# ShiqiYu/libfacedetection.train

Hardware: AMD Instinct MI355X
Metric: training images/sec, YuNet_n 320x320 bs=256/GPU (higher is better)
Workload: dtype f32; 1 GPU; YuNet_n 320x320 bs=256/GPU full training step, fp32 (64->64 backward GEMMs: two-way bf16 split -- measured against the exact-fp32 instruction: every output within 9e-6 of its tensor maximum, 50 SGD iterations end as far from the exact path as a last-bit perturbation of it does, tests/test_precision_gpu.py + profiles/r05_precision.json; the strictly-fp32 variant is timed in exact_fp32_bwd with --fu; parallelism=dp1, global_batch=256

## Files before the change

### libfacedetection.train_amd/csrc/common.h

```cpp
#pragma once
#include <hip/hip_runtime.h>
#include <stdint.h>
#include <stdlib.h>

#include "../../include/yunet_hip.h"

#define CONV_BLOCKS 1024

typedef float f32x4 __attribute__((ext_vector_type(4)));
typedef unsigned int u32x4 __attribute__((ext_vector_type(4)));
typedef unsigned int u32x2 __attribute__((ext_vector_type(2)));

#ifdef YUNET_ACT_BF16
typedef unsigned short act_t;
typedef u32x2 act_raw4;
#define ACT_SUFFIX(name) name##_bf16
#define YUNET_ACT_DTYPE YUNET_BF16
#else
typedef float act_t;
typedef u32x4 act_raw4;
#define ACT_SUFFIX(name) name
#define YUNET_ACT_DTYPE YUNET_F32
#endif
#define ACT_B ((unsigned)sizeof(act_t))
// ... 101 lines not shown
    const double mean = bn_sum_finish(bn.stats, bn.slots, C, c, r.s) * inv;
    double var = bn_sum_finish(bn.stats, bn.slots, C, C + c, r.q) * inv - mean * mean;
    var = var < 0.0 ? 0.0 : var;
    BNCoef k;
    k.mean = (float)mean;
    k.mean_lo = (float)(mean - (double)k.mean);
    k.invstd = (float)(1.0 / sqrt(var + (double)bn.eps));
    k.scale = r.gamma * k.invstd;
    k.beta = r.beta;
    return k;
}
__device__ __forceinline__ BNCoef bn_coef(const YunetBN& bn, int C, int c) {
    BNCoefRaw r = bn_coef_issue(bn, C, c);
    return bn_coef_finish(bn, C, c, r);
}
__device__ __forceinline__ void bn_table_fill(float* tab, const YunetBN& bn, int C, int tid) {
    if (tid < C) {
        const BNCoef k = bn_coef(bn, C, tid);
        tab[tid] = k.mean; tab[C + tid] = k.scale; tab[2 * C + tid] = k.beta; tab[3 * C + tid] = k.invstd;
        tab[4 * C + tid] = k.mean_lo;
    }
}
__device__ __forceinline__ void bn_table_get(const float* tab, int C, int c0, BNCoef (&k)[4]) {
#pragma unroll
    for (int i = 0; i < 4; ++i) {
        k[i].mean = tab[c0 + i]; k[i].scale = tab[C + c0 + i]; k[i].beta = tab[2 * C + c0 + i];
        k[i].invstd = tab[3 * C + c0 + i]; k[i].mean_lo = tab[4 * C + c0 + i];
    }
}

struct BNBwd {
    float mean, invstd, k1, c1, c2;
    float mean_lo, c1_lo;
};
struct BNBwdRaw {
// ... 10 lines not shown
__device__ __forceinline__ BNBwd bn_bwd_coef_finish(const YunetBN& bn, int C, int c, BNBwdRaw& r) {
    const BNCoef f = bn_coef_finish(bn, C, c, r.f);
    const double inv = 1.0 / (double)bn.count;
    BNBwd k;
    k.mean = f.mean;
    k.invstd = f.invstd;
    k.k1 = f.scale;
    const double c1 = bn_sum_finish(bn.bstats, bn.slots, C, c, r.bs) * inv;
    k.c1 = (float)c1;
    k.c1_lo = (float)(c1 - (double)k.c1);
    k.c2 = (float)(bn_sum_finish(bn.bstats, bn.slots, C, C + c, r.bq) * inv);
    k.mean_lo = f.mean_lo;
    return k;
}
__device__ __forceinline__ BNBwd bn_bwd_coef(const YunetBN& bn, int C, int c) {
    const BNCoef f = bn_coef(bn, C, c);
    const double inv = 1.0 / (double)bn.count;
    BNBwd k;
    k.mean = f.mean;
    k.invstd = f.invstd;
    k.k1 = f.scale;
    const double c1 = bn_sum(bn.bstats, bn.slots, C, c) * inv;
    k.c1 = (float)c1;
    k.c1_lo = (float)(c1 - (double)k.c1);
    k.c2 = (float)(bn_sum(bn.bstats, bn.slots, C, C + c) * inv);
    k.mean_lo = f.mean_lo;
    return k;
}

struct BNFold {
    float a, b, dh, dl;
};
__device__ __forceinline__ BNFold bn_fold(const BNBwd& k) {
    BNFold f;
    f.a = k.k1;
    f.b = (float)(-(double)k.k1 * (double)k.c2 * (double)k.invstd);
    const double D = -(double)f.a * ((double)k.c1 + (double)k.c1_lo) - (double)f.b * ((double)k.mean + (double)k.mean_lo);
    f.dh = (float)D;
    f.dl = (float)(D - (double)f.dh);
    return f;
}
__device__ __forceinline__ float bn_dz_folded(float dy, float z, float a, float b, float dh, float dl) {
// ... 176 lines not shown
```

### libfacedetection.train_amd/csrc/conv_bwd.hip

```cpp
#include "common.h"
#include "dp_route.h"
#include "dp_bwd_parts.h"

#include <type_traits>

namespace {

#define BWD_THREADS 512
#define BWD_WAVES 8

template <int CIN, int COUT, int TH, int TW, int GEMM = 0>
struct BwdGeom {
    static constexpr int HW_ = TW + 2, HH_ = TH + 2, HP = HH_ * HW_;
    static constexpr int IP = TH * TW, IMT = IP / 16;
    static constexpr int LSO = COUT + 4, LSI = CIN + 4, WS = CIN + 4, WST = COUT + 4;
    static constexpr int C4I = CIN / 4, C4O = COUT / 4;
    static constexpr int NTO = COUT / 16, NTI = CIN / 16;
    static constexpr int KSI = CIN / 4, KSO = COUT / 4;
    static constexpr int PG = BWD_THREADS / C4O;
    static constexpr int PPT = IP / PG;
    static constexpr int MB = (NTI >= 2 && (NTI * NTO < 16 || GEMM == 1)) ? 2 : 1, NB = NTO >= 2 ? 2 : 1;
    static constexpr int NGRP = (NTI / MB) * (NTO / NB);
    static constexpr int KSPLIT = BWD_WAVES / NGRP;
    static constexpr int KSTEPS = (IP / 4) / KSPLIT;
// ... 63 lines not shown
        else return y < H && x < W;
    };

    float4 pdy[G::NDZ];
    act_raw4 pz[G::NDZ], px[G::NX];
    unsigned okmask = 0;
    static_assert(!(POOLDY && PACKED), "pooled dy: unpacked levels only");
    static_assert(!POOLDY || G::NDZ <= 16, "posmask holds 16 slots");
    unsigned pid[POOLDY ? G::NDZ : 1];
    unsigned posmask = 0;
    const int Wq = W >> 1;
    const unsigned pooledbytes = (unsigned)((H >> 1) * Wq * COUT) * 4u;
    const unsigned dybytes = (unsigned)(H * W * COUT) * 4u, zbytes = (unsigned)(H * W * COUT) * ACT_B;
    const unsigned xbytes = (unsigned)(H * W * CIN) * ACT_B, dxbytes = (unsigned)(H * W * CIN) * 4u;
    constexpr int PSTEP = BWD_THREADS / G::C4O;
    auto issue = [&](int t, auto part_c) {
        constexpr int PART = decltype(part_c)::value;
        const int tid = G::LAUNDER ? opaque((int)threadIdx.x) : (int)threadIdx.x;
        const int och4 = tid % G::C4O, ich4 = tid % G::C4I;
        const int n = PACKED ? 0 : t / tiles_img, rr = t - n * tiles_img;
        const int y0 = (rr / tiles_x) * TH, x0 = (rr % tiles_x) * TW;
        const unsigned dyrange = PACKED ? (unsigned)d.N * (unsigned)d.z_img_stride * 4u : dybytes;
        const unsigned zrange = PACKED ? (unsigned)d.N * (unsigned)d.z_img_stride * ACT_B : zbytes;
        const unsigned xrange = PACKED ? (unsigned)d.N * (unsigned)d.x_img_stride * ACT_B : xbytes;
        const size_t zbase = PACKED ? (size_t)0 : (size_t)n * d.z_img_stride;
        const size_t xbase = PACKED ? (size_t)0 : (size_t)n * d.x_img_stride;
        const auto r_dy = __builtin_amdgcn_make_buffer_rsrc(
            const_cast<float*>(d.dy) + (POOLDY ? (size_t)n * (pooledbytes / 4u) : zbase), 0, POOLDY ? pooledbytes : dyrange, 0x00020000);
        const auto r_id = __builtin_amdgcn_make_buffer_rsrc(
            d.pool_idx + (POOLDY ? (size_t)n * (pooledbytes / 4u) : (size_t)0), 0,
            POOLDY ? pooledbytes / 4u : 0u, 0x00020000);
        const auto r_z = __builtin_amdgcn_make_buffer_rsrc(
            reinterpret_cast<act_t*>(const_cast<float*>(d.z)) + zbase, 0, zrange, 0x00020000);
        const auto r_x = __builtin_amdgcn_make_buffer_rsrc(
            reinterpret_cast<act_t*>(const_cast<float*>(d.x)) + xbase, 0, xrange, 0x00020000);
        if (PART <= 0) { okmask = 0; posmask = 0; }
#pragma unroll
        for (int i = 0; i < G::NDZ; ++i) {
            if (PART >= 0 && PART != 1 + (3 * i) / G::NDZ) continue;
            const int hp = tid / G::C4O + PSTEP * i;
            const int hy = hp / G::HW_, hx = hp - hy * G::HW_;
            const int y = y0 - 1 + hy, x = x0 - 1 + hx;
            bool ok;
            unsigned eo;
            if constexpr (PACKED) {
                int pn, py, px;
                ok = hp < G::HP && pk_locate(pk, y, x, pn, py, px);
                eo = (unsigned)(pn * d.z_img_stride + (py * W + px) * COUT + och4 * 4);
            } else {
                ok = hp < G::HP && (unsigned)y < (unsigned)H && (unsigned)x < (unsigned)W;
                eo = (unsigned)((y * W + x) * COUT + och4 * 4);
            }
            okmask |= ok ? (1u << i) : 0u;
            if constexpr (POOLDY) {
                const unsigned eq = (unsigned)(((y >> 1) * Wq + (x >> 1)) * COUT + och4 * 4);
                posmask |= (unsigned)(((y & 1) << 1) | (x & 1)) << (2 * i);
                const u32x4 vdy = __builtin_amdgcn_raw_buffer_load_b128(r_dy, ok ? eq * 4u : pooledbytes, 0, 0);
                pdy[i] = *reinterpret_cast<const float4*>(&vdy);
                pid[i] = __builtin_amdgcn_raw_buffer_load_b32(r_id, ok ? eq : pooledbytes, 0, 0);
            } else {
                const u32x4 vdy = __builtin_amdgcn_raw_buffer_load_b128(r_dy, ok ? eo * 4u : dyrange, 0, 0);
                pdy[i] = *reinterpret_cast<const float4*>(&vdy);
            }
            pz[i] = act_raw4{};
            if (bn_out) pz[i] = act_bufld4(r_z, ok ? eo * ACT_B : zrange);
            if constexpr (PACKED) __builtin_amdgcn_sched_barrier(0);
        }
#pragma unroll
        for (int i = 0; i < G::NX; ++i) {
            if (PART > 0) continue;
            const int ip = (tid + BWD_THREADS * i) / G::C4I;
            const int y = y0 + ip / TW, x = x0 + ip % TW;
            unsigned off;
            if constexpr (PACKED) {
                int pn, py, px;
                off = pk_locate(pk, y, x, pn, py, px)
                          ? (unsigned)(pn * d.x_img_stride + (py * W + px) * CIN + ich4 * 4) * ACT_B : xrange;
            } else {
                off = (FULL || (y < H && x < W)) ? (unsigned)((y * W + x) * CIN + ich4 * 4) * ACT_B : xbytes;
            }
            px[i] = act_bufld4(r_x, off);
            if constexpr (PACKED) __builtin_amdgcn_sched_barrier(0);
        }
    };

    using All = std::integral_constant<int, -1>;
    int t = first_tile();
    if (t < ntiles) issue(t, All{});

    if constexpr (GEMM == 1) {
        static_assert(COUT * CIN <= 8 * BWD_THREADS && (8 * BWD_THREADS) % (COUT * CIN) == 0, "8-weight groups per thread");
        const int t8 = tid % (COUT * CIN / 8);
        {
            const int co = t8 / (CIN / 8), c0 = (t8 % (CIN / 8)) * 8;
            const float4 a = *reinterpret_cast<const float4*>(d.w_pw + co * CIN + c0);
            const float4 b = *reinterpret_cast<const float4*>(d.w_pw + co * CIN + c0 + 4);
            const float w8[8] = {a.x, a.y, a.z, a.w, b.x, b.y, b.z, b.w};
            const Split8 sp = split8(w8);
            *reinterpret_cast<u32x4*>(s_w1h + co * G::WSB + c0) = sp.hi;
            *reinterpret_cast<u32x4*>(s_w1l + co * G::WSB + c0) = sp.lo;
            if (c0 == 0) s_b1[co] = d.b_pw[co];
        }
        {
            const int ci = t8 / (COUT / 8), o0 = (t8 % (COUT / 8)) * 8;
            float w8[8];
#pragma unroll
            for (int j = 0; j < 8; ++j) w8[j] = d.w_pw[(o0 + j) * CIN + ci];
            const Split8 sp = split8(w8);
            *reinterpret_cast<u32x4*>(s_w1th + ci * G::WSTB + o0) = sp.hi;
            *reinterpret_cast<u32x4*>(s_w1tl + ci * G::WSTB + o0) = sp.lo;
        }
    } else {
        staged_table<COUT * CIN, BWD_THREADS>(d.w_pw, tid, [&](int i, float w) {
            s_w1[(i / CIN) * G::WS + (i % CIN)] = w;
            if (i % CIN == 0) s_w1[(i / CIN) * G::WS + CIN] = d.b_pw[i / CIN];
            s_w1t[(i % CIN) * G::WST + (i / CIN)] = w;
        });
    }
    staged_table<COUT * 9, BWD_THREADS>(d.w_dw, tid, [&](int i, float w) { s_w2[(i % 9) * COUT + i / 9] = w; });
    for (int c = tid; c < COUT; c += BWD_THREADS) {
        if (bn_out) {
            const BNFold f = bn_fold(bn_bwd_coef(d.out_bn, COUT, c));
            s_co[c] = f.a; s_co[COUT + c] = f.b; s_co[2 * COUT + c] = f.dh; s_co[3 * COUT + c] = f.dl;
        } else {
            s_co[c] = d.dy_scale ? d.dy_scale[c] : 1.0f;
            s_co[COUT + c] = 0.f; s_co[2 * COUT + c] = 0.f; s_co[3 * COUT + c] = 0.f;
        }
    }
    for (int c = tid; c < CIN; c += BWD_THREADS) {
        if (bn_in) {
            const BNCoef k = bn_coef(d.in_bn, CIN, c);
            s_ci[c] = k.mean; s_ci[CIN + c] = k.scale; s_ci[2 * CIN + c] = k.beta;
            s_ci[3 * CIN + c] = k.invstd; s_ci[4 * CIN + c] = k.mean_lo;
        } else {
            s_ci[c] = 0.f; s_ci[CIN + c] = 1.f; s_ci[2 * CIN + c] = 0.f; s_ci[3 * CIN + c] = 1.f;
            s_ci[4 * CIN + c] = 0.f;
        }
    }
    __syncthreads();

    const int cq = tid % G::C4O, pg = tid / G::C4O;
    const int vtx = pg % TW, vr0 = (pg / TW) * G::PPT;
    float4 gw2[9];
#pragma unroll
    for (int t = 0; t < 9; ++t) gw2[t] = make_float4(0, 0, 0, 0);
    float4 gb2 = make_float4(0, 0, 0, 0), gb1 = make_float4(0, 0, 0, 0);
// ... 43 lines not shown
            }
            if constexpr (PACKED) {
                for (int ip = tid; ip < G::IP; ip += BWD_THREADS) {
                    int pn, py, px;
                    s_in[ip] = pk_locate(pk, y0 + ip / TW, x0 + ip % TW, pn, py, px) ? 1 : 0;
                }
            }
#pragma unroll
            for (int i = 0; i < G::NX; ++i) {
                const int ip = (tid + BWD_THREADS * i) / G::C4I;
                *reinterpret_cast<float4*>(s_a + ip * G::LSI + ich4 * 4) = act_unpack(px[i]);
            }
        }
        __syncthreads();
        const bool more = t + (int)gridDim.x < ntiles && pf_on;
        if (SPREAD && more) issue(t + gridDim.x, std::integral_constant<int, 0>{});

        if constexpr (GEMM == 1) {
            if (!(abl & 1)) {
#pragma unroll 1
                for (int mi = 0; mi < G::MPW; ++mi) {
                    const int mt = wid * G::MPW + mi;
                    f32x4 acc[G::NTO];
#pragma unroll
                    for (int nt = 0; nt < G::NTO; ++nt) acc[nt] = f32x4{0.f, 0.f, 0.f, 0.f};
                    const float* arow = s_a + (mt * 16 + l15) * G::LSI + 8 * g;
                    const float* crow = s_ci + 8 * g;
                    const __bf16* bh = s_w1h + l15 * G::WSB + 8 * g;
                    const __bf16* bl = s_w1l + l15 * G::WSB + 8 * g;
#pragma unroll
                    for (int kb = 0; kb < CIN / 32; ++kb) {
// ... 75 lines not shown
                }
                float bias_pw[G::NTO];
#pragma unroll
                for (int nt = 0; nt < G::NTO; ++nt) bias_pw[nt] = s_w1[(nt * 16 + (G::LAUNDER ? opaque(l15) : l15)) * G::WS + CIN];
#pragma unroll
                for (int r = 0; r < 4; ++r) {
                    const int ip = mt * 16 + 4 * g + r;
                    const bool in = inside(ip, y0 + ip / TW, x0 + ip % TW);
#pragma unroll
                    for (int nt = 0; nt < G::NTO; ++nt)
                        s_pb[ip * G::LSO + nt * 16 + l15] = in ? acc[nt][r] + bias_pw[nt] : 0.0f;
                }
            }
        }
        __syncthreads();
        if (SPREAD && more) issue(t + gridDim.x, std::integral_constant<int, 1>{});

        if (!(abl & 2)) {
            const int tv = G::LAUNDER ? opaque((int)threadIdx.x) : (int)threadIdx.x;
            const int cq = tv % G::C4O, pg = tv / G::C4O;
            const int vtx = pg % TW, vr0 = (pg / TW) * G::PPT;
            const float* zb = s_dz + (vr0 * G::HW_ + vtx) * G::LSO + cq * 4;
            float* pb = s_pb + (vr0 * TW + vtx) * G::LSO + cq * 4;
            const float* wb = s_w2 + cq * 4;
            float4 pv[G::PPT], dp[G::PPT];
#pragma unroll
            for (int r = 0; r < G::PPT; ++r) {
                pv[r] = *reinterpret_cast<const float4*>(pb + r * TW * G::LSO);
                dp[r] = make_float4(0, 0, 0, 0);
            }
#pragma unroll
// ... 18 lines not shown
                            gb2.x += z4.x; gb2.y += z4.y; gb2.z += z4.z; gb2.w += z4.w;
                        }
                    }
                }
                if (G::PPT > 1) __builtin_amdgcn_sched_barrier(0);
            }
#pragma unroll
            for (int r = 0; r < G::PPT; ++r) {
                const bool in = inside((vr0 + r) * TW + vtx, y0 + vr0 + r, x0 + vtx);
                if (!in) dp[r] = make_float4(0, 0, 0, 0);
                gb1.x += dp[r].x; gb1.y += dp[r].y; gb1.z += dp[r].z; gb1.w += dp[r].w;
                *reinterpret_cast<float4*>(pb + r * TW * G::LSO) = dp[r];
            }
        }
        __syncthreads();
        if (SPREAD) { if (more) issue(t + gridDim.x, std::integral_constant<int, 2>{}); }
        else if (more) issue(t + gridDim.x, All{});

        if constexpr (GEMM == 1) {
            if (!(abl & 4)) {
                static_assert(GEMM == 0 || (G::MB == 2 && G::NB == 2), "bf16 dW1: 2x2 interleaved tiles");
                const float* ap = s_a + (w1_kslice * G::KPX + 8 * g) * G::LSI + w1_ci0 + 2 * l15;
                const float* bp = s_pb + (w1_kslice * G::KPX + 8 * g) * G::LSO + w1_co0 + 2 * l15;
                float am[2], as_[2], ab[2];
#pragma unroll
                for (int j = 0; j < 2; ++j) {
                    const int ca = w1_ci0 + 2 * (G::LAUNDER ? opaque(l15) : l15) + j;
                    am[j] = s_ci[ca]; as_[j] = s_ci[CIN + ca]; ab[j] = s_ci[2 * CIN + ca];
                }
#pragma unroll 1
                for (int kb = 0; kb < G::KPX / 32; ++kb) {
                    Split8 sd0, sd1;
// ... 65 lines not shown
                    if constexpr (NPART > 1) {
                        part[s % NPART] = mfma16(a, bv[0], part[s % NPART]);
                    } else {
#pragma unroll
                        for (int i = 0; i < G::NB; ++i)
                            gw1[j * G::NB + i] = mfma16(a, bv[i], gw1[j * G::NB + i]);
                    }
                }
            }
            if constexpr (NPART > 1) {
                static_assert(NPART == 1 || G::KSTEPS % 4 == 0, "partial accumulators: whole rounds of four k-steps");
#pragma unroll
                for (int r = 0; r < 4; ++r) gw1[0][r] += (part[0][r] + part[1][r]) + (part[2][r] + part[3][r]);
            }
        }
        if (SPREAD && more) issue(t + gridDim.x, std::integral_constant<int, 3>{});
        f32x4 da[G::MPW][G::NTI];
#pragma unroll
        for (int mi = 0; mi < G::MPW; ++mi)
#pragma unroll
            for (int nt = 0; nt < G::NTI; ++nt) da[mi][nt] = f32x4{0.f, 0.f, 0.f, 0.f};
        if constexpr (GEMM == 1) {
            if (!(abl & 8)) {
#pragma unroll
                for (int mi = 0; mi < G::MPW; ++mi) {
                    const float* prow = s_pb + ((wid * G::MPW + mi) * 16 + l15) * G::LSO + 8 * g;
                    const __bf16* wh = s_w1th + l15 * G::WSTB + 8 * g;
                    const __bf16* wl = s_w1tl + l15 * G::WSTB + 8 * g;
#pragma unroll
                    for (int kb = 0; kb < COUT / 32; ++kb) {
                        float p8[8];
// ... 241 lines not shown
```

### libfacedetection.train_amd/csrc/conv_bwd_ew.hip

```cpp
#include "common.h"
#include "bwd_grid.h"

namespace {

__global__ __launch_bounds__(256) void stem_bwd_kernel(const float* __restrict__ img,
                                                       const act_t* __restrict__ z,
                                                       const float* __restrict__ dy, YunetBN bn,
                                                       float* __restrict__ partials, int N, int H,
                                                       int W) {
    constexpr int PH = 2 * SB_TH + 1;
    constexpr int PW4 = (2 * SB_TW + 8) / 4;
    constexpr int PWS = PW4 * 4 + 1;
    constexpr int NLD = (3 * PH * PW4 + 255) / 256;
    constexpr int DZS = 20;
    constexpr int PATCH_F = ((3 * PH * PWS + 3) / 4) * 4;
    constexpr int DZT_F = SB_TH * SB_TW * DZS;
    constexpr int ALL_F = (PATCH_F + DZT_F) > 256 * 33 ? (PATCH_F + DZT_F) : 256 * 33;
    __shared__ __attribute__((aligned(16))) float s_all[ALL_F];
    float* s_patch = s_all;
    float* s_dzt = s_all + PATCH_F;
    __shared__ float s_k[4][16];
    const int tid = threadIdx.x;
    const int Ho = H / 2, Wo = W / 2;
    if (tid < 16) {
// ... 300 lines not shown
        else atomic_add_f64(bn_slot(DST, SLOTS, C) + which * C + c, v);              \
    }
    UPADD_FLUSH(bsa, (dxa ? bna.bstats : nullptr), bna.slots)
    UPADD_FLUSH(bsb, bnb.bstats, bnb.slots)
#undef UPADD_FLUSH
}

template <bool DET = false>
__global__ __launch_bounds__(256) void upadd_bwd_coarse_kernel(const act_t* __restrict__ zb, YunetBN bnb,
                                                               const float* __restrict__ dout, float* __restrict__ dxb,
                                                               int acc_b, int N, int H, int W, int C) {
    const int C4 = C / 4, Hb = H / 2, Wb = W / 2;
    const long long total = (long long)N * Hb * Wb * C4;
    const int c4 = threadIdx.x % C4;
    __shared__ float s_tb[5 * 64];
    bn_table_fill(s_tb, bnb, C, threadIdx.x);
    __syncthreads();
    BNCoef kb[4];
    bn_table_get(s_tb, C, c4 * 4, kb);
    double bsb[8];
#pragma unroll
    for (int i = 0; i < 8; ++i) bsb[i] = 0.0;
    for (long long e = (long long)blockIdx.x * 256 + threadIdx.x; e < total; e += (long long)gridDim.x * 256) {
        long long pix = e / C4;
        const int bx = (int)(pix % Wb);
        pix /= Wb;
        const int by = (int)(pix % Hb), n = (int)(pix / Hb);
        const size_t off0 = (((size_t)n * H + 2 * by) * W + 2 * bx) * C + c4 * 4;
        const size_t offb = (((size_t)n * Hb + by) * Wb + bx) * C + c4 * 4;
        const float4 g0 = *reinterpret_cast<const float4*>(dout + off0);
        const float4 g1 = *reinterpret_cast<const float4*>(dout + off0 + C);
        const float4 g2 = *reinterpret_cast<const float4*>(dout + off0 + (size_t)W * C);
        const float4 g3 = *reinterpret_cast<const float4*>(dout + off0 + (size_t)W * C + C);
        const float4 zb4 = act_ld4(zb + offb);
        float4 old = make_float4(0.f, 0.f, 0.f, 0.f);
        if (acc_b) old = *reinterpret_cast<const float4*>(dxb + offb);
        const float sum[4] = {((0.f + g0.x) + g1.x) + g2.x + g3.x, ((0.f + g0.y) + g1.y) + g2.y + g3.y,
                              ((0.f + g0.z) + g1.z) + g2.z + g3.z, ((0.f + g0.w) + g1.w) + g2.w + g3.w};
        const float zbv[4] = {zb4.x, zb4.y, zb4.z, zb4.w};
        float ob[4];
#pragma unroll
        for (int i = 0; i < 4; ++i) {
            const bool on = bnrelu(zbv[i], kb[i].mean, kb[i].scale, kb[i].beta) > 0.0f;
            ob[i] = on ? sum[i] : 0.0f;
            const float xh = on ? bn_center(zbv[i], kb[i].mean, kb[i].mean_lo) * kb[i].invstd : 0.0f;
            bsb[i] += (double)ob[i];
            bsb[4 + i] += (double)(ob[i] * xh);
        }
        float4 v = make_float4(ob[0], ob[1], ob[2], ob[3]);
        if (acc_b) { v.x += old.x; v.y += old.y; v.z += old.z; v.w += old.w; }
        *reinterpret_cast<float4*>(dxb + offb) = v;
    }
    __shared__ double red[256 * 8];
#pragma unroll
    for (int i = 0; i < 8; ++i) red[threadIdx.x * 8 + i] = bsb[i];
    __syncthreads();
    if ((int)threadIdx.x < 2 * C && bnb.bstats) {
        const int which = threadIdx.x / C, c = threadIdx.x % C;
        const int q = c >> 2, kk = (c & 3) + 4 * which;
        double v = 0.0;
        for (int p = 0; p < 256 / C4; ++p) v += red[(p * C4 + q) * 8 + kk];
        if constexpr (DET) bn_det_add(bnb.bstats, C, which * C + c, v);
        else atomic_add_f64(bn_slot(bnb.bstats, bnb.slots, C) + which * C + c, v);
    }
}

// ... 34 lines not shown
extern "C" int ACT_SUFFIX(yunet_pool_bwd)(const float* z, const YunetBN* bn, const float* dy_out, float* dx,
                                          int accumulate, int N, int H, int W, int C, void* stream) {
    return ACT_SUFFIX(yunet_pool_bwd_add)(z, bn, dy_out, nullptr, dx, accumulate, N, H, W, C, stream);
}

extern "C" int ACT_SUFFIX(yunet_upadd_bwd)(const float* za, const YunetBN* bna, const float* zb,
                                           const YunetBN* bnb, const float* dout, float* dxa, int accumulate_a,
                                           float* dxb, int accumulate_b, int N, int H, int W, int C,
                                           void* stream) {
    if ((H & 1) || (W & 1) || (C & 3) || (256 % (C / 4)) || C > 64) return YUNET_EINVAL;
    const long long total = (long long)N * (H / 2) * (W / 2) * (C / 4);
    if ((YUNET_DET_ROWS(bnb->det_rows) && bnb->bstats) || (dxa && YUNET_DET_ROWS(bna->det_rows) && bna->bstats)) {
#ifndef YUNET_ACT_BF16
        if (!bnb->bstats || !bn_det_fits(*bnb, ew_grid(total)) || (dxa && (!bna->bstats || !bn_det_fits(*bna, ew_grid(total)))))
            return YUNET_EINVAL;
        if (!dxa)
            hipLaunchKernelGGL(upadd_bwd_coarse_kernel<true>, dim3(ew_grid(total)), dim3(256), 0, (hipStream_t)stream,
                               reinterpret_cast<const act_t*>(zb), *bnb, dout, dxb, accumulate_b, N, H, W, C);
        else
            hipLaunchKernelGGL(upadd_bwd_kernel<true>, dim3(ew_grid(total)), dim3(256), 0, (hipStream_t)stream,
                               reinterpret_cast<const act_t*>(za), *bna, reinterpret_cast<const act_t*>(zb), *bnb, dout, dxa,
                               accumulate_a, dxb, accumulate_b, N, H, W, C);
        return hip_status();
#else
        return YUNET_EINVAL;
#endif
    }
    if (!dxa && yunet_options().upadd_coarse) {
        hipLaunchKernelGGL(upadd_bwd_coarse_kernel<false>, dim3(ew_grid(total)), dim3(256), 0, (hipStream_t)stream,
                           reinterpret_cast<const act_t*>(zb), *bnb, dout, dxb, accumulate_b, N, H, W, C);
        return hip_status();
    }
    hipLaunchKernelGGL(upadd_bwd_kernel<false>, dim3(ew_grid(total)), dim3(256), 0, (hipStream_t)stream,
                       reinterpret_cast<const act_t*>(za), *bna, reinterpret_cast<const act_t*>(zb), *bnb, dout, dxa,
                       accumulate_a, dxb, accumulate_b, N, H, W, C);
    return hip_status();
}
```

### libfacedetection.train_amd/csrc/conv_fwd.hip

```cpp
#include <cstdlib>

#include <stdlib.h>

#include "dp_route.h"

namespace {

#define STEM_TW 32
#define STEM_TH 16
#define STEM_PX 2
__global__ __launch_bounds__(256) void stem_fwd_kernel(const float* __restrict__ img,
                                                       const float* __restrict__ w,
                                                       const float* __restrict__ b,
                                                       act_t* __restrict__ z,
                                                       double* __restrict__ stats, int N, int H,
                                                       int W) {
    constexpr int PH = 2 * STEM_TH + 1;
    constexpr int PW4 = (2 * STEM_TW + 8) / 4;
    constexpr int PWS = PW4 * 4 + 1;
    constexpr int NLD = (3 * PH * PW4 + 255) / 256;
    __shared__ float s_patch[3 * PH * PWS];
    __shared__ __attribute__((aligned(16))) float s_w[27][16];
    __shared__ double s_stat[32];
    const int tid = threadIdx.x;
// ... 159 lines not shown
    const int l15 = lane & 15, g = lane >> 4;
    const int H = d.H, W = d.W;
    const bool bn_in = d.in_transform == YUNET_T_BNRELU;

    const int lch4 = tid % G::C4I;
    const int tiles_x = ((PACKED ? pk.CW : W) + TW - 1) / TW, tiles_y = ((PACKED ? pk.CH : H) + TH - 1) / TH;
    const int tiles_img = tiles_x * tiles_y;
    const int ntiles = PACKED ? tiles_img : d.N * tiles_img;

    act_raw4 pre[G::NLD];
    const bool z_f32 = YUNET_ACT_DTYPE == YUNET_F32 || (COUT == 16 && d.z_dtype == YUNET_F32);
    const unsigned ZB = z_f32 ? 4u : ACT_B;
    const unsigned xbytes = (unsigned)(H * W * CIN) * ACT_B, zbytes = (unsigned)(H * W * COUT) * ZB;
    constexpr int PSTEP = 256 / G::C4I;
    constexpr int HSTEP_Y = PSTEP / G::HW_, HSTEP_X = PSTEP % G::HW_;
    auto issue = [&](int t) {
        const int n = PACKED ? 0 : t / tiles_img, rr = t - n * tiles_img;
        const int y0 = (rr / tiles_x) * TH, x0 = (rr % tiles_x) * TW;
        const unsigned xrange = PACKED ? (unsigned)d.N * (unsigned)d.x_img_stride * ACT_B : xbytes;
        const auto r_x = __builtin_amdgcn_make_buffer_rsrc(
            reinterpret_cast<act_t*>(const_cast<float*>(d.x)) + (PACKED ? (size_t)0 : (size_t)n * d.x_img_stride), 0,
            xrange, 0x00020000);
        int hp = tid / G::C4I;
        int hy = hp / G::HW_, hx = hp - hy * G::HW_;
#pragma unroll
        for (int i = 0; i < G::NLD; ++i) {
            const int y = y0 - 1 + hy, x = x0 - 1 + hx;
            bool ok;
            unsigned off;
            if constexpr (PACKED) {
                int pn, py, px;
                ok = hp < G::HP && pk_locate(pk, y, x, pn, py, px);
                off = ok ? (unsigned)(pn * d.x_img_stride + (py * W + px) * CIN + lch4 * 4) * ACT_B : xrange;
            } else {
                ok = hp < G::HP && (unsigned)y < (unsigned)H && (unsigned)x < (unsigned)W;
                off = ok ? (unsigned)((y * W + x) * CIN + lch4 * 4) * ACT_B : xbytes;
            }
            pre[i] = act_bufld4(r_x, off);
            hp += PSTEP; hy += HSTEP_Y; hx += HSTEP_X;
            if (hx >= G::HW_) { hx -= G::HW_; ++hy; }
        }
    };
    int t = first_tile();
    if (t < ntiles) issue(t);

    constexpr bool BF16_MMA = YUNET_ACT_DTYPE == YUNET_BF16 && CIN % 32 == 0;
    constexpr int WSB = CIN + 8;
    __bf16* s_w1b = reinterpret_cast<__bf16*>(s_w1);
    constexpr bool SPLIT3 = YUNET_ACT_DTYPE == YUNET_F32 && CIN % 32 == 0;
    constexpr int NCH = CIN / 8;
    __bf16* s_w1p = reinterpret_cast<__bf16*>(s_w1);
    if constexpr (SPLIT3) {
        staged_table<COUT * CIN, 256>(d.w_pw, tid, [&](int i, float w) {
            const int co = i / CIN, ci = i % CIN;
            const __bf16 h = (__bf16)w;
            const float r1 = w - (float)h;
            const __bf16 m = (__bf16)r1;
            const __bf16 l = (__bf16)(r1 - (float)m);
            const int at = co * CIN + (((ci >> 3) ^ (co & (NCH - 1))) << 3) + (ci & 7);
            s_w1p[at] = h; s_w1p[COUT * CIN + at] = m; s_w1p[2 * COUT * CIN + at] = l;
        });
    } else if constexpr (BF16_MMA) {
        staged_table<COUT * CIN, 256>(d.w_pw, tid, [&](int i, float w) { s_w1b[(i / CIN) * WSB + (i % CIN)] = (__bf16)w; });
    } else {
        staged_table<COUT * CIN, 256>(d.w_pw, tid, [&](int i, float w) { s_w1[(i / CIN) * G::WS + (i % CIN)] = w; });
    }
    staged_table<COUT * 9, 256>(d.w_dw, tid, [&](int i, float w) { s_w2[(i % 9) * COUT + i / 9] = w; });
    for (int i = tid; i < COUT; i += 256) s_b2[i] = d.b_dw[i];
    for (int c = tid; c < CIN; c += 256) {
        BNCoef k{0.f, 1.f, 0.f, 1.f};
        if (bn_in) k = bn_coef(d.in_bn, CIN, c);
        s_coef[c] = k.mean;
        s_coef[CIN + c] = k.scale;
        s_coef[2 * CIN + c] = k.beta;
    }
    float bias_pw[G::NT];
#pragma unroll
    for (int nt = 0; nt < G::NT; ++nt) bias_pw[nt] = d.b_pw[nt * 16 + l15];
    const int cq = tid % G::C4O, pg = tid / G::C4O;
    const int dtx = pg % TW, r0 = (pg / TW) * G::RPT;
    double st[8];
#pragma unroll
    for (int i = 0; i < 8; ++i) st[i] = 0.0;
    float sg[4] = {1.f, 1.f, 1.f, 1.f};
    if constexpr (POOL) {
#pragma unroll
        for (int i = 0; i < 4; ++i) {
            const float gm = d.out_bn.gamma[cq * 4 + i];
            sg[i] = gm > 0.0f ? 1.0f : (gm < 0.0f ? -1.0f : 0.0f);
        }
    }
    __syncthreads();

    const float relu_floor = bn_in ? 0.0f : -__builtin_inff();

    unsigned long long pc[4] = {0, 0, 0, 0}, c0 = 0;
    const bool prof = (unsigned long long)d.prof >= 64ull;
    const unsigned abl = (unsigned long long)d.prof < 64ull ? (unsigned)(unsigned long long)d.prof : 0u;
    for (; t < ntiles; t += gridDim.x) {
        if (prof) c0 = clock64();
        const int n = PACKED ? 0 : t / tiles_img, rr = t - n * tiles_img;
        const int y0 = (rr / tiles_x) * TH, x0 = (rr % tiles_x) * TW;
        {
            const float4 cm = *reinterpret_cast<const float4*>(s_coef + lch4 * 4);
            const float4 cs = *reinterpret_cast<const float4*>(s_coef + CIN + lch4 * 4);
// ... 2 lines not shown
#pragma unroll
            for (int i = 0; i < G::NLD; ++i) {
                const int hp = hp0 + PSTEP * i;
                if ((i + 1) * PSTEP <= G::MP || hp < G::MP) {
                    float4 v = act_unpack(pre[i]);
                    v.x = fmaxf(fmaf(v.x - cm.x, cs.x, cb.x), relu_floor);
                    v.y = fmaxf(fmaf(v.y - cm.y, cs.y, cb.y), relu_floor);
                    v.z = fmaxf(fmaf(v.z - cm.z, cs.z, cb.z), relu_floor);
                    v.w = fmaxf(fmaf(v.w - cm.w, cs.w, cb.w), relu_floor);
                    *reinterpret_cast<float4*>(buf + hp * G::LS + lch4 * 4) = v;
                }
            }
        }
        __syncthreads();
        if (prof) { const unsigned long long c = clock64(); pc[0] += c - c0; c0 = c; }
        if (t + (int)gridDim.x < ntiles && !(abl & 8)) issue(t + gridDim.x);
        auto store_p = [&](int mt, const f32x4 (&acc)[G::NT]) {
#pragma unroll
        for (int r = 0; r < 4; ++r) {
            const int hp = mt * 16 + 4 * g + r;
            const int hy = hp / G::HW_, hx = hp - hy * G::HW_;
            const int y = y0 - 1 + hy, x = x0 - 1 + hx;
            int pn, py, px;
            const bool in = hp < G::HP && (PACKED ? pk_locate(pk, y, x, pn, py, px)
                                                 : (y >= 0 && y < H && x >= 0 && x < W));
#pragma unroll
            for (int nt = 0; nt < G::NT; ++nt)
                buf[hp * G::LS + nt * 16 + l15] = in ? acc[nt][r] + bias_pw[nt] : 0.0f;
        }
        };
        for (int mt = wid; mt < ((abl & 1) ? 0 : G::MT); mt += 4) {
// ... 412 lines not shown
```

Before: 60390 images/sec.

## Overlap kernel prologue weight/BN-stat loads with first-tile prefetch

Restructures the prologues of the forward and backward conv kernels and the upadd backward kernel. Weight, bias and BN-statistic global loads are now issued into registers first, together with the first tile's activation prefetch, and only then finished and written to shared memory. This overlaps their latencies instead of serialising several dependent load rounds. Out-of-range first tiles are handled with a 'live' predicate so the loads are always issued. The change also adds early returns for empty launches, and the added register pressure could affect occupancy.

Measured after the change: 60600 images/sec, median of 6. No clear change (+0.3%).

```diff
diff --git a/libfacedetection.train_amd/csrc/common.h b/libfacedetection.train_amd/csrc/common.h
--- a/libfacedetection.train_amd/csrc/common.h
+++ b/libfacedetection.train_amd/csrc/common.h
@@ -139,11 +139,20 @@
     BNCoefRaw r = bn_coef_issue(bn, C, c);
     return bn_coef_finish(bn, C, c, r);
 }
+__device__ __forceinline__ BNCoefRaw bn_table_issue(const YunetBN& bn, int C, int tid) {
+    return bn_coef_issue(bn, C, tid < C ? tid : 0);
+}
+__device__ __forceinline__ void bn_table_finish(float* tab, const YunetBN& bn, int C, int tid, BNCoefRaw& r) {
+    if (tid < C) {
+        const BNCoef k = bn_coef_finish(bn, C, tid, r);
+        tab[tid] = k.mean; tab[C + tid] = k.scale; tab[2 * C + tid] = k.beta; tab[3 * C + tid] = k.invstd;
+        tab[4 * C + tid] = k.mean_lo;
+    }
+}
 __device__ __forceinline__ void bn_table_fill(float* tab, const YunetBN& bn, int C, int tid) {
     if (tid < C) {
-        const BNCoef k = bn_coef(bn, C, tid);
-        tab[tid] = k.mean; tab[C + tid] = k.scale; tab[2 * C + tid] = k.beta; tab[3 * C + tid] = k.invstd;
-        tab[4 * C + tid] = k.mean_lo;
+        BNCoefRaw r = bn_coef_issue(bn, C, tid);
+        bn_table_finish(tab, bn, C, tid, r);
     }
 }
 __device__ __forceinline__ void bn_table_get(const float* tab, int C, int c0, BNCoef (&k)[4]) {
@@ -184,18 +193,8 @@
     return k;
 }
 __device__ __forceinline__ BNBwd bn_bwd_coef(const YunetBN& bn, int C, int c) {
-    const BNCoef f = bn_coef(bn, C, c);
-    const double inv = 1.0 / (double)bn.count;
-    BNBwd k;
-    k.mean = f.mean;
-    k.invstd = f.invstd;
-    k.k1 = f.scale;
-    const double c1 = bn_sum(bn.bstats, bn.slots, C, c) * inv;
-    k.c1 = (float)c1;
-    k.c1_lo = (float)(c1 - (double)k.c1);
-    k.c2 = (float)(bn_sum(bn.bstats, bn.slots, C, C + c) * inv);
-    k.mean_lo = f.mean_lo;
-    return k;
+    BNBwdRaw r = bn_bwd_coef_issue(bn, C, c);
+    return bn_bwd_coef_finish(bn, C, c, r);
 }
 
 struct BNFold {
diff --git a/libfacedetection.train_amd/csrc/conv_bwd.hip b/libfacedetection.train_amd/csrc/conv_bwd.hip
--- a/libfacedetection.train_amd/csrc/conv_bwd.hip
+++ b/libfacedetection.train_amd/csrc/conv_bwd.hip
@@ -101,8 +101,9 @@
     const unsigned dybytes = (unsigned)(H * W * COUT) * 4u, zbytes = (unsigned)(H * W * COUT) * ACT_B;
     const unsigned xbytes = (unsigned)(H * W * CIN) * ACT_B, dxbytes = (unsigned)(H * W * CIN) * 4u;
     constexpr int PSTEP = BWD_THREADS / G::C4O;
-    auto issue = [&](int t, auto part_c) {
+    auto issue = [&](int t, auto part_c, auto live_c) {
         constexpr int PART = decltype(part_c)::value;
+        const bool live = live_c;
         const int tid = G::LAUNDER ? opaque((int)threadIdx.x) : (int)threadIdx.x;
         const int och4 = tid % G::C4O, ich4 = tid % G::C4I;
         const int n = PACKED ? 0 : t / tiles_img, rr = t - n * tiles_img;
@@ -132,10 +133,10 @@
             unsigned eo;
             if constexpr (PACKED) {
                 int pn, py, px;
-                ok = hp < G::HP && pk_locate(pk, y, x, pn, py, px);
+                ok = live && hp < G::HP && pk_locate(pk, y, x, pn, py, px);
                 eo = (unsigned)(pn * d.z_img_stride + (py * W + px) * COUT + och4 * 4);
             } else {
-                ok = hp < G::HP && (unsigned)y < (unsigned)H && (unsigned)x < (unsigned)W;
+                ok = live && hp < G::HP && (unsigned)y < (unsigned)H && (unsigned)x < (unsigned)W;
                 eo = (unsigned)((y * W + x) * COUT + och4 * 4);
             }
             okmask |= ok ? (1u << i) : 0u;
@@ -149,8 +150,7 @@
                 const u32x4 vdy = __builtin_amdgcn_raw_buffer_load_b128(r_dy, ok ? eo * 4u : dyrange, 0, 0);
                 pdy[i] = *reinterpret_cast<const float4*>(&vdy);
             }
-            pz[i] = act_raw4{};
-            if (bn_out) pz[i] = act_bufld4(r_z, ok ? eo * ACT_B : zrange);
+            pz[i] = act_bufld4(r_z, (ok && bn_out) ? eo * ACT_B : zrange);
             if constexpr (PACKED) __builtin_amdgcn_sched_barrier(0);
         }
 #pragma unroll
@@ -161,10 +161,10 @@
             unsigned off;
             if constexpr (PACKED) {
                 int pn, py, px;
-                off = pk_locate(pk, y, x, pn, py, px)
+                off = (live && pk_locate(pk, y, x, pn, py, px))
                           ? (unsigned)(pn * d.x_img_stride + (py * W + px) * CIN + ich4 * 4) * ACT_B : xrange;
             } else {
-                off = (FULL || (y < H && x < W)) ? (unsigned)((y * W + x) * CIN + ich4 * 4) * ACT_B : xbytes;
+                off = (live && (FULL || (y < H && x < W))) ? (unsigned)((y * W + x) * CIN + ich4 * 4) * ACT_B : xbytes;
             }
             px[i] = act_bufld4(r_x, off);
             if constexpr (PACKED) __builtin_amdgcn_sched_barrier(0);
@@ -172,51 +172,78 @@
     };
 
     using All = std::integral_constant<int, -1>;
+    static_assert(COUT <= BWD_THREADS && CIN <= BWD_THREADS, "one coefficient per thread");
     int t = first_tile();
-    if (t < ntiles) issue(t, All{});
-
+    constexpr int W1N = (COUT * CIN + BWD_THREADS - 1) / BWD_THREADS, W2N = (COUT * 9 + BWD_THREADS - 1) / BWD_THREADS;
+    float w1v[GEMM == 1 ? 1 : W1N], w2v[W2N];
+    float4 w8a, w8b;
+    float w8t[8];
+    const int t8 = GEMM == 1 ? tid % (COUT * CIN / 8) : 0;
     if constexpr (GEMM == 1) {
         static_assert(COUT * CIN <= 8 * BWD_THREADS && (8 * BWD_THREADS) % (COUT * CIN) == 0, "8-weight groups per thread");
-        const int t8 = tid % (COUT * CIN / 8);
+        const int co = t8 / (CIN / 8), c0 = (t8 % (CIN / 8)) * 8;
+        w8a = *reinterpret_cast<const float4*>(d.w_pw + co * CIN + c0);
+        w8b = *reinterpret_cast<const float4*>(d.w_pw + co * CIN + c0 + 4);
+        const int ci = t8 / (COUT / 8), o0 = (t8 % (COUT / 8)) * 8;
+#pragma unroll
+        for (int j = 0; j < 8; ++j) w8t[j] = d.w_pw[(o0 + j) * CIN + ci];
+    } else {
+        staged_issue<COUT * CIN, BWD_THREADS>(d.w_pw, tid, w1v);
+    }
+    staged_issue<COUT * 9, BWD_THREADS>(d.w_dw, tid, w2v);
+    const float b1v = d.b_pw[tid < COUT ? tid : COUT - 1];
+    float dsv = 1.0f;
+    BNBwdRaw oraw;
+    BNCoefRaw iraw;
+    if (bn_out) {
+        if (tid < COUT) oraw = bn_bwd_coef_issue(d.out_bn, COUT, tid);
+    } else if (d.dy_scale) {
+        dsv = d.dy_scale[tid < COUT ? tid : COUT - 1];
+    }
+    if (bn_in && tid < CIN) iraw = bn_coef_issue(d.in_bn, CIN, tid);
+    {
+        const bool live = t < ntiles;
+        issue(live ? t : 0, All{}, live);
+    }
+    __builtin_amdgcn_sched_barrier(0);
+
+    if constexpr (GEMM == 1) {
         {
             const int co = t8 / (CIN / 8), c0 = (t8 % (CIN / 8)) * 8;
-            const float4 a = *reinterpret_cast<const float4*>(d.w_pw + co * CIN + c0);
-            const float4 b = *reinterpret_cast<const float4*>(d.w_pw + co * CIN + c0 + 4);
-            const float w8[8] = {a.x, a.y, a.z, a.w, b.x, b.y, b.z, b.w};
+            const float w8[8] = {w8a.x, w8a.y, w8a.z, w8a.w, w8b.x, w8b.y, w8b.z, w8b.w};
             const Split8 sp = split8(w8);
             *reinterpret_cast<u32x4*>(s_w1h + co * G::WSB + c0) = sp.hi;
             *reinterpret_cast<u32x4*>(s_w1l + co * G::WSB + c0) = sp.lo;
-            if (c0 == 0) s_b1[co] = d.b_pw[co];
         }
         {
             const int ci = t8 / (COUT / 8), o0 = (t8 % (COUT / 8)) * 8;
-            float w8[8];
-#pragma unroll
-            for (int j = 0; j < 8; ++j) w8[j] = d.w_pw[(o0 + j) * CIN + ci];
-            const Split8 sp = split8(w8);
+            const Split8 sp = split8(w8t);
             *reinterpret_cast<u32x4*>(s_w1th + ci * G::WSTB + o0) = sp.hi;
             *reinterpret_cast<u32x4*>(s_w1tl + ci * G::WSTB + o0) = sp.lo;
         }
+        if (tid < COUT) s_b1[tid] = b1v;
     } else {
-        staged_table<COUT * CIN, BWD_THREADS>(d.w_pw, tid, [&](int i, float w) {
+        staged_put<COUT * CIN, BWD_THREADS>(tid, w1v, [&](int i, float w) {
             s_w1[(i / CIN) * G::WS + (i % CIN)] = w;
-            if (i % CIN == 0) s_w1[(i / CIN) * G::WS + CIN] = d.b_pw[i / CIN];
             s_w1t[(i % CIN) * G::WST + (i / CIN)] = w;
         });
-    }
-    staged_table<COUT * 9, BWD_THREADS>(d.w_dw, tid, [&](int i, float w) { s_w2[(i % 9) * COUT + i / 9] = w; });
-    for (int c = tid; c < COUT; c += BWD_THREADS) {
+        if (tid < COUT) s_w1[tid * G::WS + CIN] = b1v;
+    }
+    staged_put<COUT * 9, BWD_THREADS>(tid, w2v, [&](int i, float w) { s_w2[(i % 9) * COUT + i / 9] = w; });
+    if (tid < COUT) {
+        const int c = tid;
         if (bn_out) {
-            const BNFold f = bn_fold(bn_bwd_coef(d.out_bn, COUT, c));
+            const BNFold f = bn_fold(bn_bwd_coef_finish(d.out_bn, COUT, c, oraw));
             s_co[c] = f.a; s_co[COUT + c] = f.b; s_co[2 * COUT + c] = f.dh; s_co[3 * COUT + c] = f.dl;
         } else {
-            s_co[c] = d.dy_scale ? d.dy_scale[c] : 1.0f;
+            s_co[c] = dsv;
             s_co[COUT + c] = 0.f; s_co[2 * COUT + c] = 0.f; s_co[3 * COUT + c] = 0.f;
         }
     }
-    for (int c = tid; c < CIN; c += BWD_THREADS) {
+    if (tid < CIN) {
+        const int c = tid;
         if (bn_in) {
-            const BNCoef k = bn_coef(d.in_bn, CIN, c);
+            const BNCoef k = bn_coef_finish(d.in_bn, CIN, c, iraw);
             s_ci[c] = k.mean; s_ci[CIN + c] = k.scale; s_ci[2 * CIN + c] = k.beta;
             s_ci[3 * CIN + c] = k.invstd; s_ci[4 * CIN + c] = k.mean_lo;
         } else {
@@ -290,7 +317,7 @@
         }
         __syncthreads();
         const bool more = t + (int)gridDim.x < ntiles && pf_on;
-        if (SPREAD && more) issue(t + gridDim.x, std::integral_constant<int, 0>{});
+        if (SPREAD && more) issue(t + gridDim.x, std::integral_constant<int, 0>{}, std::true_type{});
 
         if constexpr (GEMM == 1) {
             if (!(abl & 1)) {
@@ -396,7 +423,7 @@
             }
         }
         __syncthreads();
-        if (SPREAD && more) issue(t + gridDim.x, std::integral_constant<int, 1>{});
+        if (SPREAD && more) issue(t + gridDim.x, std::integral_constant<int, 1>{}, std::true_type{});
 
         if (!(abl & 2)) {
             const int tv = G::LAUNDER ? opaque((int)threadIdx.x) : (int)threadIdx.x;
@@ -445,8 +472,8 @@
             }
         }
         __syncthreads();
-        if (SPREAD) { if (more) issue(t + gridDim.x, std::integral_constant<int, 2>{}); }
-        else if (more) issue(t + gridDim.x, All{});
+        if (SPREAD) { if (more) issue(t + gridDim.x, std::integral_constant<int, 2>{}, std::true_type{}); }
+        else if (more) issue(t + gridDim.x, All{}, std::true_type{});
 
         if constexpr (GEMM == 1) {
             if (!(abl & 4)) {
@@ -542,7 +569,7 @@
                 for (int r = 0; r < 4; ++r) gw1[0][r] += (part[0][r] + part[1][r]) + (part[2][r] + part[3][r]);
             }
         }
-        if (SPREAD && more) issue(t + gridDim.x, std::integral_constant<int, 3>{});
+        if (SPREAD && more) issue(t + gridDim.x, std::integral_constant<int, 3>{}, std::true_type{});
         f32x4 da[G::MPW][G::NTI];
 #pragma unroll
         for (int mi = 0; mi < G::MPW; ++mi)
diff --git a/libfacedetection.train_amd/csrc/conv_bwd_ew.hip b/libfacedetection.train_amd/csrc/conv_bwd_ew.hip
--- a/libfacedetection.train_amd/csrc/conv_bwd_ew.hip
+++ b/libfacedetection.train_amd/csrc/conv_bwd_ew.hip
@@ -338,25 +338,26 @@
     const long long total = (long long)N * Hb * Wb * C4;
     const int c4 = threadIdx.x % C4;
     __shared__ float s_tb[5 * 64];
-    bn_table_fill(s_tb, bnb, C, threadIdx.x);
-    __syncthreads();
     BNCoef kb[4];
-    bn_table_get(s_tb, C, c4 * 4, kb);
     double bsb[8];
 #pragma unroll
     for (int i = 0; i < 8; ++i) bsb[i] = 0.0;
-    for (long long e = (long long)blockIdx.x * 256 + threadIdx.x; e < total; e += (long long)gridDim.x * 256) {
+    auto fetch = [&](long long e, float4 (&g)[4], act_raw4& zr) {
         long long pix = e / C4;
         const int bx = (int)(pix % Wb);
         pix /= Wb;
         const int by = (int)(pix % Hb), n = (int)(pix / Hb);
         const size_t off0 = (((size_t)n * H + 2 * by) * W + 2 * bx) * C + c4 * 4;
-        const size_t offb = (((size_t)n * Hb + by) * Wb + bx) * C + c4 * 4;
-        const float4 g0 = *reinterpret_cast<const float4*>(dout + off0);
-        const float4 g1 = *reinterpret_cast<const float4*>(dout + off0 + C);
-        const float4 g2 = *reinterpret_cast<const float4*>(dout + off0 + (size_t)W * C);
-        const float4 g3 = *reinterpret_cast<const float4*>(dout + off0 + (size_t)W * C + C);
-        const float4 zb4 = act_ld4(zb + offb);
+        g[0] = *reinterpret_cast<const float4*>(dout + off0);
+        g[1] = *reinterpret_cast<const float4*>(dout + off0 + C);
+        g[2] = *reinterpret_cast<const float4*>(dout + off0 + (size_t)W * C);
+        g[3] = *reinterpret_cast<const float4*>(dout + off0 + (size_t)W * C + C);
+        zr = *reinterpret_cast<const act_raw4*>(zb + e * 4);
+    };
+    auto mask = [&](long long e, const float4 (&g)[4], const act_raw4 zr) {
+        const size_t offb = (size_t)e * 4;
+        const float4 g0 = g[0], g1 = g[1], g2 = g[2], g3 = g[3];
+        const float4 zb4 = act_unpack(zr);
         float4 old = make_float4(0.f, 0.f, 0.f, 0.f);
         if (acc_b) old = *reinterpret_cast<const float4*>(dxb + offb);
         const float sum[4] = {((0.f + g0.x) + g1.x) + g2.x + g3.x, ((0.f + g0.y) + g1.y) + g2.y + g3.y,
@@ -374,6 +375,22 @@
         float4 v = make_float4(ob[0], ob[1], ob[2], ob[3]);
         if (acc_b) { v.x += old.x; v.y += old.y; v.z += old.z; v.w += old.w; }
         *reinterpret_cast<float4*>(dxb + offb) = v;
+    };
+    const long long e0 = (long long)blockIdx.x * 256 + threadIdx.x, estep = (long long)gridDim.x * 256;
+    BNCoefRaw raw = bn_table_issue(bnb, C, threadIdx.x);
+    float4 fg[4];
+    act_raw4 fz;
+    fetch(e0 < total ? e0 : 0, fg, fz);
+    __builtin_amdgcn_sched_barrier(0);
+    bn_table_finish(s_tb, bnb, C, threadIdx.x, raw);
+    __syncthreads();
+    bn_table_get(s_tb, C, c4 * 4, kb);
+    if (e0 < total) mask(e0, fg, fz);
+    for (long long e = e0 + estep; e < total; e += estep) {
+        float4 g[4];
+        act_raw4 zr;
+        fetch(e, g, zr);
+        mask(e, g, zr);
     }
     __shared__ double red[256 * 8];
 #pragma unroll
@@ -438,6 +455,7 @@
 #ifndef YUNET_ACT_BF16
         if (!bnb->bstats || !bn_det_fits(*bnb, ew_grid(total)) || (dxa && (!bna->bstats || !bn_det_fits(*bna, ew_grid(total)))))
             return YUNET_EINVAL;
+        if (!dxa && total <= 0) return 0;
         if (!dxa)
             hipLaunchKernelGGL(upadd_bwd_coarse_kernel<true>, dim3(ew_grid(total)), dim3(256), 0, (hipStream_t)stream,
                                reinterpret_cast<const act_t*>(zb), *bnb, dout, dxb, accumulate_b, N, H, W, C);
@@ -451,6 +469,7 @@
 #endif
     }
     if (!dxa && yunet_options().upadd_coarse) {
+        if (total <= 0) return 0;
         hipLaunchKernelGGL(upadd_bwd_coarse_kernel<false>, dim3(ew_grid(total)), dim3(256), 0, (hipStream_t)stream,
                            reinterpret_cast<const act_t*>(zb), *bnb, dout, dxb, accumulate_b, N, H, W, C);
         return hip_status();
diff --git a/libfacedetection.train_amd/csrc/conv_fwd.hip b/libfacedetection.train_amd/csrc/conv_fwd.hip
--- a/libfacedetection.train_amd/csrc/conv_fwd.hip
+++ b/libfacedetection.train_amd/csrc/conv_fwd.hip
@@ -1,6 +1,8 @@
 #include <cstdlib>
 
 #include <stdlib.h>
+
+#include <type_traits>
 
 #include "dp_route.h"
 
@@ -197,7 +199,8 @@
     const unsigned xbytes = (unsigned)(H * W * CIN) * ACT_B, zbytes = (unsigned)(H * W * COUT) * ZB;
     constexpr int PSTEP = 256 / G::C4I;
     constexpr int HSTEP_Y = PSTEP / G::HW_, HSTEP_X = PSTEP % G::HW_;
-    auto issue = [&](int t) {
+    auto issue = [&](int t, auto live_c) {
+        const bool live = live_c;
         const int n = PACKED ? 0 : t / tiles_img, rr = t - n * tiles_img;
         const int y0 = (rr / tiles_x) * TH, x0 = (rr % tiles_x) * TW;
         const unsigned xrange = PACKED ? (unsigned)d.N * (unsigned)d.x_img_stride * ACT_B : xbytes;
@@ -213,10 +216,10 @@
             unsigned off;
             if constexpr (PACKED) {
                 int pn, py, px;
-                ok = hp < G::HP && pk_locate(pk, y, x, pn, py, px);
+                ok = live && hp < G::HP && pk_locate(pk, y, x, pn, py, px);
                 off = ok ? (unsigned)(pn * d.x_img_stride + (py * W + px) * CIN + lch4 * 4) * ACT_B : xrange;
             } else {
-                ok = hp < G::HP && (unsigned)y < (unsigned)H && (unsigned)x < (unsigned)W;
+                ok = live && hp < G::HP && (unsigned)y < (unsigned)H && (unsigned)x < (unsigned)W;
                 off = ok ? (unsigned)((y * W + x) * CIN + lch4 * 4) * ACT_B : xbytes;
             }
             pre[i] = act_bufld4(r_x, off);
@@ -225,7 +228,6 @@
         }
     };
     int t = first_tile();
-    if (t < ntiles) issue(t);
 
     constexpr bool BF16_MMA = YUNET_ACT_DTYPE == YUNET_BF16 && CIN % 32 == 0;
     constexpr int WSB = CIN + 8;
@@ -233,8 +235,32 @@
     constexpr bool SPLIT3 = YUNET_ACT_DTYPE == YUNET_F32 && CIN % 32 == 0;
     constexpr int NCH = CIN / 8;
     __bf16* s_w1p = reinterpret_cast<__bf16*>(s_w1);
+    static_assert(COUT <= 256 && CIN <= 256, "one coefficient per thread");
+    constexpr int W1N = (COUT * CIN + 255) / 256, W2N = (COUT * 9 + 255) / 256;
+    float w1v[W1N], w2v[W2N];
+    staged_issue<COUT * CIN, 256>(d.w_pw, tid, w1v);
+    staged_issue<COUT * 9, 256>(d.w_dw, tid, w2v);
+    const float b2v = d.b_dw[tid < COUT ? tid : COUT - 1];
+    float bias_pw[G::NT];
+#pragma unroll
+    for (int nt = 0; nt < G::NT; ++nt) bias_pw[nt] = d.b_pw[nt * 16 + l15];
+    const int cq = tid % G::C4O, pg = tid / G::C4O;
+    const int dtx = pg % TW, r0 = (pg / TW) * G::RPT;
+    float gm[4] = {1.f, 1.f, 1.f, 1.f};
+    if constexpr (POOL) {
+#pragma unroll
+        for (int i = 0; i < 4; ++i) gm[i] = d.out_bn.gamma[cq * 4 + i];
+    }
+    BNCoefRaw iraw;
+    if (bn_in && tid < CIN) iraw = bn_coef_issue(d.in_bn, CIN, tid);
+    {
+        const bool live = t < ntiles;
+        issue(live ? t : 0, live);
+    }
+    __builtin_amdgcn_sched_barrier(0);
+
     if constexpr (SPLIT3) {
-        staged_table<COUT * CIN, 256>(d.w_pw, tid, [&](int i, float w) {
+        staged_put<COUT * CIN, 256>(tid, w1v, [&](int i, float w) {
             const int co = i / CIN, ci = i % CIN;
             const __bf16 h = (__bf16)w;
             const float r1 = w - (float)h;
@@ -244,34 +270,27 @@
             s_w1p[at] = h; s_w1p[COUT * CIN + at] = m; s_w1p[2 * COUT * CIN + at] = l;
         });
     } else if constexpr (BF16_MMA) {
-        staged_table<COUT * CIN, 256>(d.w_pw, tid, [&](int i, float w) { s_w1b[(i / CIN) * WSB + (i % CIN)] = (__bf16)w; });
+        staged_put<COUT * CIN, 256>(tid, w1v, [&](int i, float w) { s_w1b[(i / CIN) * WSB + (i % CIN)] = (__bf16)w; });
     } else {
-        staged_table<COUT * CIN, 256>(d.w_pw, tid, [&](int i, float w) { s_w1[(i / CIN) * G::WS + (i % CIN)] = w; });
-    }
-    staged_table<COUT * 9, 256>(d.w_dw, tid, [&](int i, float w) { s_w2[(i % 9) * COUT + i / 9] = w; });
-    for (int i = tid; i < COUT; i += 256) s_b2[i] = d.b_dw[i];
-    for (int c = tid; c < CIN; c += 256) {
+        staged_put<COUT * CIN, 256>(tid, w1v, [&](int i, float w) { s_w1[(i / CIN) * G::WS + (i % CIN)] = w; });
+    }
+    staged_put<COUT * 9, 256>(tid, w2v, [&](int i, float w) { s_w2[(i % 9) * COUT + i / 9] = w; });
+    if (tid < COUT) s_b2[tid] = b2v;
+    if (tid < CIN) {
+        const int c = tid;
         BNCoef k{0.f, 1.f, 0.f, 1.f};
-        if (bn_in) k = bn_coef(d.in_bn, CIN, c);
+        if (bn_in) k = bn_coef_finish(d.in_bn, CIN, c, iraw);
         s_coef[c] = k.mean;
         s_coef[CIN + c] = k.scale;
         s_coef[2 * CIN + c] = k.beta;
     }
-    float bias_pw[G::NT];
-#pragma unroll
-    for (int nt = 0; nt < G::NT; ++nt) bias_pw[nt] = d.b_pw[nt * 16 + l15];
-    const int cq = tid % G::C4O, pg = tid / G::C4O;
-    const int dtx = pg % TW, r0 = (pg / TW) * G::RPT;
     double st[8];
 #pragma unroll
     for (int i = 0; i < 8; ++i) st[i] = 0.0;
     float sg[4] = {1.f, 1.f, 1.f, 1.f};
     if constexpr (POOL) {
 #pragma unroll
-        for (int i = 0; i < 4; ++i) {
-            const float gm = d.out_bn.gamma[cq * 4 + i];
-            sg[i] = gm > 0.0f ? 1.0f : (gm < 0.0f ? -1.0f : 0.0f);
-        }
+        for (int i = 0; i < 4; ++i) sg[i] = gm[i] > 0.0f ? 1.0f : (gm[i] < 0.0f ? -1.0f : 0.0f);
     }
     __syncthreads();
 
@@ -304,7 +323,7 @@
         }
         __syncthreads();
         if (prof) { const unsigned long long c = clock64(); pc[0] += c - c0; c0 = c; }
-        if (t + (int)gridDim.x < ntiles && !(abl & 8)) issue(t + gridDim.x);
+        if (t + (int)gridDim.x < ntiles && !(abl & 8)) issue(t + gridDim.x, std::true_type{});
         auto store_p = [&](int mt, const f32x4 (&acc)[G::NT]) {
 #pragma unroll
         for (int r = 0; r < 4; ++r) {
```
